# AlexIoannides/bodywork-mlops-demo

Measured on NVIDIA H100. Metric: train rows/sec (N x 128 least-squares fit), higher is better.
Workload: dtype bf16x2 (hi+lo) MMA operands, f32 accumulate, f64 fold+solve

## Files before the change

### bodywork-mlops-demo_b200/csrc/b2_internal.cuh

```cuda
#pragma once
#include <cuda.h>
#include <cuda_bf16.h>
#include <cuda_runtime.h>
#include <stdint.h>
#include <stdio.h>
#include <string.h>

#include <type_traits>

#include "../../include/b2gram.h"

namespace b2 {

constexpr int kMaxD = B2_MAX_D;
constexpr int kMaxS = kMaxD + 2;
constexpr int kKernelEventPairs = 64;
constexpr int kMaxRanks = 8;
constexpr size_t kXchgSlotDoubles = (size_t)kMaxS * kMaxS;
constexpr size_t kXchgDataDoubles = 2 * kMaxRanks * kXchgSlotDoubles;
constexpr size_t kXchgBytes = kXchgDataDoubles * sizeof(double) + 256;

constexpr int kTcRows = 64;
constexpr int kTcM = 128;
constexpr int kTcN = 144;
constexpr int kTcAccCols = 2 * kTcN;
constexpr int kTcAccElems = kTcM * kTcAccCols;
constexpr int kTcSums = 3;

constexpr int kNStats = 10;
constexpr int kGradOut = kMaxD + 1;
constexpr int kRfBeta = 0;
constexpr int kRfB0 = kMaxD;
constexpr int kRfMean = kMaxD + 1;
constexpr int kRfPrevBeta = 2 * kMaxD + 1;
constexpr int kRfPrevB0 = 3 * kMaxD + 1;
constexpr int kRfStep = 3 * kMaxD + 2;
constexpr int kRfGrad = 3 * kMaxD + 3;
constexpr int kRfDoubles = kRfGrad + kGradOut;
constexpr int kOutRefineStep = 2 * kMaxD + 3;
constexpr int kOutRefineGuard = 2 * kMaxD + 4;

inline int narrow_dp(int d) { return d <= 1 ? 1 : d <= 2 ? 2 : d <= 4 ? 4 : d <= 8 ? 8 : 16; }

void set_error(const char* fmt, ...);

#define B2_CUDA(call)                                                                      \
  do {                                                                                     \
    cudaError_t e_ = (call);                                                               \
    if (e_ != cudaSuccess) {                                                               \
// ... 132 lines not shown
```

### bodywork-mlops-demo_b200/csrc/gram_tc.cu

```cuda
#include <cuda_bf16.h>
#include <stdlib.h>

#include "b2_internal.cuh"
#include "b2_ptx.cuh"
#include "b2_shift.cuh"
#include "b2_xchg.cuh"

namespace b2 {
namespace {

constexpr int kConsumerWGs = 2;
constexpr int kXformWarps = 8;
constexpr int kThreads = 128 * (kConsumerWGs + 2);
constexpr int kFirstXformWarp = 4 * kConsumerWGs;
constexpr int kTmaWarp = kFirstXformWarp;
constexpr int kEWarp = kFirstXformWarp + 1;
static_assert(kFirstXformWarp + kXformWarps == kThreads / 32, "warp roles");
constexpr int kProducers = kXformWarps;
constexpr int kConsumerWarps = 4 * kConsumerWGs;
constexpr int kAccRegs = kTcN / 2;
constexpr int kKGroups = kTcRows / 8;
constexpr uint32_t kRawStageBytes = kTcRows * kMaxD * 4;
constexpr uint32_t kOpSBO = 128;
constexpr uint32_t kOpLBO = (16 + 2 + 16) * kOpSBO;
constexpr uint32_t kOpEOff = 16 * kOpSBO;
constexpr uint32_t kOpLoOff = 18 * kOpSBO;
constexpr uint32_t kOpStageBytes = kKGroups * kOpLBO;
constexpr int kMaxPack = 5;
constexpr uint32_t kYStageBytes = kTcRows * kMaxPack * 4;
constexpr uint32_t kMStageBytes = 384;
static_assert(kMStageBytes >= kTcRows * kMaxPack && kMStageBytes % 128 == 0 && kYStageBytes % 128 == 0, "stage alignment");

template <bool RAWB>
struct TcGeo {
  static constexpr int kRawStages = RAWB ? 4 : 3;
  static constexpr int kOpStages = RAWB ? 2 : 3;
  static constexpr int kAhead = RAWB ? kRawStages - 2 : kRawStages - 1;
  static constexpr uint32_t kOffRaw = 0;
  static constexpr uint32_t kOffOp = kOffRaw + kRawStages * kRawStageBytes;
  static constexpr uint32_t kOffY = kOffOp + kOpStages * kOpStageBytes;
  static constexpr uint32_t kOffMask = kOffY + kRawStages * kYStageBytes;
  static constexpr uint32_t kOffBar = kOffMask + kRawStages * kMStageBytes;
  static constexpr int kNumBars = 2 * kRawStages + 2 * kOpStages;
// ... 18 lines not shown
__device__ __forceinline__ void tma_load_1d(uint32_t dst, const CUtensorMap* tm, int c0, uint32_t bar) {
  asm volatile(
      "cp.async.bulk.tensor.1d.shared::cluster.global.mbarrier::complete_tx::bytes.L2::cache_hint"
      " [%0], [%1, {%3}], [%2], %4;" ::"r"(dst),
      "l"(reinterpret_cast<uint64_t>(tm)), "r"(bar), "r"(c0), "l"(kEvictFirst)
      : "memory");
}
__device__ __forceinline__ void tma_prefetch_desc(const CUtensorMap* tm) {
  asm volatile("prefetch.tensormap [%0];" ::"l"(reinterpret_cast<uint64_t>(tm)) : "memory");
}

__device__ __forceinline__ uint64_t make_smem_desc(uint32_t addr) {
  return (uint64_t)((addr & 0x3FFFFu) >> 4) | ((uint64_t)(kOpLBO >> 4) << 16) | ((uint64_t)(kOpSBO >> 4) << 32);
}
__device__ __forceinline__ void wgmma_fence() { asm volatile("wgmma.fence.sync.aligned;" ::: "memory"); }
__device__ __forceinline__ void wgmma_commit() { asm volatile("wgmma.commit_group.sync.aligned;" ::: "memory"); }
template <int N>
__device__ __forceinline__ void wgmma_wait() { asm volatile("wgmma.wait_group.sync.aligned %0;" ::"n"(N) : "memory"); }
template <int N>
__device__ __forceinline__ void fence_regs(float (&r)[N]) {
#pragma unroll
  for (int i = 0; i < N; ++i) asm volatile("" : "+f"(r[i])::"memory");
}
__device__ __forceinline__ void wgmma_m64n144k16(float (&d)[72], uint64_t adesc, uint64_t bdesc, uint32_t scale_d) {
  asm volatile(
      "{\n\t.reg .pred p;\n\t"
      "setp.ne.b32 p, %74, 0;\n\t"
      "wgmma.mma_async.sync.aligned.m64n144k16.f32.bf16.bf16 "
      "{%0, %1, %2, %3, %4, %5, %6, %7, %8, %9, %10, %11, "
      " %12, %13, %14, %15, %16, %17, %18, %19, %20, %21, %22, %23, "
      " %24, %25, %26, %27, %28, %29, %30, %31, %32, %33, %34, %35, "
      " %36, %37, %38, %39, %40, %41, %42, %43, %44, %45, %46, %47, "
      " %48, %49, %50, %51, %52, %53, %54, %55, %56, %57, %58, %59, "
      " %60, %61, %62, %63, %64, %65, %66, %67, %68, %69, %70, %71}, "
      "%72, %73, p, 1, 1, 0, 0;\n\t}"
      : "+f"(d[0]), "+f"(d[1]), "+f"(d[2]), "+f"(d[3]), "+f"(d[4]), "+f"(d[5]), "+f"(d[6]), "+f"(d[7]),
        "+f"(d[8]), "+f"(d[9]), "+f"(d[10]), "+f"(d[11]), "+f"(d[12]), "+f"(d[13]), "+f"(d[14]), "+f"(d[15]),
        "+f"(d[16]), "+f"(d[17]), "+f"(d[18]), "+f"(d[19]), "+f"(d[20]), "+f"(d[21]), "+f"(d[22]), "+f"(d[23]),
        "+f"(d[24]), "+f"(d[25]), "+f"(d[26]), "+f"(d[27]), "+f"(d[28]), "+f"(d[29]), "+f"(d[30]), "+f"(d[31]),
        "+f"(d[32]), "+f"(d[33]), "+f"(d[34]), "+f"(d[35]), "+f"(d[36]), "+f"(d[37]), "+f"(d[38]), "+f"(d[39]),
        "+f"(d[40]), "+f"(d[41]), "+f"(d[42]), "+f"(d[43]), "+f"(d[44]), "+f"(d[45]), "+f"(d[46]), "+f"(d[47]),
        "+f"(d[48]), "+f"(d[49]), "+f"(d[50]), "+f"(d[51]), "+f"(d[52]), "+f"(d[53]), "+f"(d[54]), "+f"(d[55]),
        "+f"(d[56]), "+f"(d[57]), "+f"(d[58]), "+f"(d[59]), "+f"(d[60]), "+f"(d[61]), "+f"(d[62]), "+f"(d[63]),
        "+f"(d[64]), "+f"(d[65]), "+f"(d[66]), "+f"(d[67]), "+f"(d[68]), "+f"(d[69]), "+f"(d[70]), "+f"(d[71])
      : "l"(adesc), "l"(bdesc), "r"(scale_d));
}
__device__ __forceinline__ void wgmma_m64n128k16_bmn(float* d, uint64_t adesc, uint64_t bdesc, uint32_t scale_d) {
  asm volatile(
      "{\n\t.reg .pred p;\n\t"
      "setp.ne.b32 p, %66, 0;\n\t"
      "wgmma.mma_async.sync.aligned.m64n128k16.f32.bf16.bf16 "
      "{%0, %1, %2, %3, %4, %5, %6, %7, %8, %9, %10, %11, %12, %13, %14, %15, "
      " %16, %17, %18, %19, %20, %21, %22, %23, %24, %25, %26, %27, %28, %29, %30, %31, "
      " %32, %33, %34, %35, %36, %37, %38, %39, %40, %41, %42, %43, %44, %45, %46, %47, "
      " %48, %49, %50, %51, %52, %53, %54, %55, %56, %57, %58, %59, %60, %61, %62, %63}, "
      "%64, %65, p, 1, 1, 0, 1;\n\t}"
      : "+f"(d[0]), "+f"(d[1]), "+f"(d[2]), "+f"(d[3]), "+f"(d[4]), "+f"(d[5]), "+f"(d[6]), "+f"(d[7]),
        "+f"(d[8]), "+f"(d[9]), "+f"(d[10]), "+f"(d[11]), "+f"(d[12]), "+f"(d[13]), "+f"(d[14]), "+f"(d[15]),
        "+f"(d[16]), "+f"(d[17]), "+f"(d[18]), "+f"(d[19]), "+f"(d[20]), "+f"(d[21]), "+f"(d[22]), "+f"(d[23]),
        "+f"(d[24]), "+f"(d[25]), "+f"(d[26]), "+f"(d[27]), "+f"(d[28]), "+f"(d[29]), "+f"(d[30]), "+f"(d[31]),
        "+f"(d[32]), "+f"(d[33]), "+f"(d[34]), "+f"(d[35]), "+f"(d[36]), "+f"(d[37]), "+f"(d[38]), "+f"(d[39]),
        "+f"(d[40]), "+f"(d[41]), "+f"(d[42]), "+f"(d[43]), "+f"(d[44]), "+f"(d[45]), "+f"(d[46]), "+f"(d[47]),
        "+f"(d[48]), "+f"(d[49]), "+f"(d[50]), "+f"(d[51]), "+f"(d[52]), "+f"(d[53]), "+f"(d[54]), "+f"(d[55]),
        "+f"(d[56]), "+f"(d[57]), "+f"(d[58]), "+f"(d[59]), "+f"(d[60]), "+f"(d[61]), "+f"(d[62]), "+f"(d[63])
      : "l"(adesc), "l"(bdesc), "r"(scale_d));
}
__device__ __forceinline__ void wgmma_m64n16k16(float* d, uint64_t adesc, uint64_t bdesc, uint32_t scale_d) {
  asm volatile(
      "{\n\t.reg .pred p;\n\t"
      "setp.ne.b32 p, %10, 0;\n\t"
      "wgmma.mma_async.sync.aligned.m64n16k16.f32.bf16.bf16 "
      "{%0, %1, %2, %3, %4, %5, %6, %7}, "
      "%8, %9, p, 1, 1, 0, 0;\n\t}"
      : "+f"(d[0]), "+f"(d[1]), "+f"(d[2]), "+f"(d[3]), "+f"(d[4]), "+f"(d[5]), "+f"(d[6]), "+f"(d[7])
      : "l"(adesc), "l"(bdesc), "r"(scale_d));
}
constexpr uint32_t kRawBoxBytes = kTcRows * 64 * 2;
__device__ __forceinline__ uint64_t make_raw_desc(uint32_t addr) {
  return (uint64_t)((addr & 0x3FFFFu) >> 4) | ((uint64_t)(kRawBoxBytes >> 4) << 16) | ((uint64_t)(1024u >> 4) << 32) |
         (1ull << 62);
}

__device__ __forceinline__ void st_shared_v4(uint32_t addr, const uint32_t (&v)[4]) {
  asm volatile("st.shared.v4.b32 [%0], {%1, %2, %3, %4};" ::"r"(addr), "r"(v[0]), "r"(v[1]), "r"(v[2]), "r"(v[3])
               : "memory");
}
__device__ __forceinline__ uint32_t lane_id() {
  uint32_t l;
  asm volatile("mov.u32 %0, %%laneid;" : "=r"(l));
  return l;
}
__device__ __forceinline__ void st_shared_f64(uint32_t addr, double v) {
  asm volatile("st.shared.f64 [%0], %1;" ::"r"(addr), "d"(v) : "memory");
}
__device__ __forceinline__ double ld_shared_f64(uint32_t addr) {
  double v;
  asm volatile("ld.shared.f64 %0, [%1];" : "=d"(v) : "r"(addr) : "memory");
  return v;
}
__device__ __forceinline__ void red_add_f64(double* p, double v) {
  asm volatile("red.global.add.f64 [%0], %1;" ::"l"(p), "d"(v) : "memory");
}
__device__ __forceinline__ void st_shared_u16(uint32_t addr, uint32_t v) {
  asm volatile("st.shared.u16 [%0], %1;" ::"r"(addr), "h"((unsigned short)v) : "memory");
}
__device__ __forceinline__ void split2(float v0, float v1, uint32_t& hi, uint32_t& lo) {
  const __nv_bfloat162 h = __floats2bfloat162_rn(v0, v1);
  hi = *reinterpret_cast<const uint32_t*>(&h);
  const float h0 = __uint_as_float(hi << 16), h1 = __uint_as_float(hi & 0xffff0000u);
  const __nv_bfloat162 l = __floats2bfloat162_rn(v0 - h0, v1 - h1);
  lo = *reinterpret_cast<const uint32_t*>(&l);
}

constexpr int kRedElems = kTcAccElems + kTcSums;

__device__ __forceinline__ void tc_reduce_range(const double* part, int n_ctas, double* red, int e0, int e1,
                                                double* quarter) {
  const int epb = blockDim.x >> 2;
  const int e = threadIdx.x % epb, q = threadIdx.x / epb;
  const int per = (n_ctas + 3) / 4;
  const int c0 = q * per, c1 = (c0 + per < n_ctas) ? c0 + per : n_ctas;
  for (int base = e0; base < e1; base += epb) {
    const int idx = base + e;
    if (idx < e1) {
      const bool sum = idx >= kTcAccElems;
      const double* src = sum ? part + (size_t)n_ctas * kTcAccElems + (idx - kTcAccElems) : part + idx;
      const size_t stride = sum ? kTcSums : kTcAccElems;
      double acc[8] = {0.0, 0.0, 0.0, 0.0, 0.0, 0.0, 0.0, 0.0};
      int c = c0;
      for (; c + 8 <= c1; c += 8) {
#pragma unroll
        for (int u = 0; u < 8; ++u) acc[u] += __ldcg(src + (size_t)(c + u) * stride);
      }
      for (; c < c1; ++c) acc[0] += __ldcg(src + (size_t)c * stride);
      quarter[q * epb + e] = ((acc[0] + acc[1]) + (acc[2] + acc[3])) + ((acc[4] + acc[5]) + (acc[6] + acc[7]));
    }
    __syncthreads();
    if (q == 0 && idx < e1) red[idx] = ((quarter[e] + quarter[epb + e]) + quarter[2 * epb + e]) + quarter[3 * epb + e];
    __syncthreads();
  }
}

__device__ __forceinline__ void grid_barrier(unsigned int* ctr) {
  __syncthreads();
  if (threadIdx.x == 0) {
    __threadfence();
    atomicAdd(ctr, 1u);
    const uint64_t t0 = globaltimer_ns();
    unsigned int seen;
    do {
      asm volatile("ld.acquire.gpu.global.u32 %0, [%1];" : "=r"(seen) : "l"(ctr) : "memory");
      if (seen < gridDim.x) {
        __nanosleep(40);
        if (globaltimer_ns() - t0 > 4000000000ull) __trap();
      }
    } while (seen < gridDim.x);
    __threadfence();
  }
  __syncthreads();
}

__device__ __forceinline__ double tc_fold_value(const double* red, const double* c, int d, int pack, int idx) {
  const int dp = d + 2;
  const int a = min(idx / dp, idx % dp), b = max(idx / dp, idx % dp);
  auto D1 = [&](int i, int j) { return __ldcg(red + (size_t)j * kTcM + i); };
  auto D2 = [&](int i, int j) { return __ldcg(red + (size_t)(kTcN + j) * kTcM + i); };
  auto s1 = [&](int i) {
    double t = 0.0;
    for (int blk = 0; blk < pack; ++blk) t += D1(blk * d + i, 128 + 3 * blk) + D2(blk * d + i, 128 + 3 * blk);
    return t;
  };
  auto sxy = [&](int i) {
    double t = 0.0;
    for (int blk = 0; blk < pack; ++blk) {
      const int r = blk * d + i, e = 128 + 3 * blk;
      t += D1(r, e + 1) + D1(r, e + 2) + D2(r, e + 1) + D2(r, e + 2);
    }
    return t;
  };
  auto G = [&](int i, int j) {
    double g = 0.0;
    for (int blk = 0; blk < pack; ++blk) {
      const int ia = blk * d + i, ib = blk * d + j;
      g += 0.5 * (D1(ia, ib) + D1(ib, ia)) + D2(ia, ib) + D2(ib, ia);
    }
    return g;
  };
  return unshift_entry(a, b, d, c, G, s1, sxy, __ldcg(red + kTcAccElems + 2), __ldcg(red + kTcAccElems + 0),
                       __ldcg(red + kTcAccElems + 1));
}

template <typename T, int DFIX, bool SPLIT, bool RAWB = false>
__global__ void __launch_bounds__(kThreads, 1)
gram_tc_kernel(const __grid_constant__ CUtensorMap tmX, const __grid_constant__ CUtensorMap tmY,
               const __grid_constant__ CUtensorMap tmM, int y_map_2d, int has_mask, int keep,
               int64_t n_rows, int d_arg, int pack, int d_orig, const float* __restrict__ shift,
               int chunk_tiles, double* __restrict__ part, uint32_t wait_ns, uint32_t dbg_arg) {
#ifdef B2_DEV_KNOBS
  const uint32_t dbg = dbg_arg;
#else
  constexpr uint32_t dbg = 0u;
  (void)dbg_arg;
#endif
  using G = TcGeo<RAWB>;
  constexpr int kRawStages = G::kRawStages, kOpStages = G::kOpStages;
  constexpr uint32_t kOffRaw = G::kOffRaw, kOffOp = G::kOffOp, kOffY = G::kOffY, kOffMask = G::kOffMask;
  const int d = DFIX ? DFIX : d_arg;
  extern __shared__ uint8_t smem_raw[];
  const uint32_t sbase = (smem_u32(smem_raw) + 1023u) & ~1023u;
  uint8_t* smem = smem_raw + (sbase - smem_u32(smem_raw));
  const int warp = threadIdx.x >> 5;
  const int lane = threadIdx.x & 31;

  const uint32_t bar_raw_full = sbase + G::kOffBar;
  const uint32_t bar_raw_empty = bar_raw_full + 8 * kRawStages;
// ... 11 lines not shown
      mbar_init(bar_raw_full + 8 * s, 1);
      mbar_init(bar_raw_empty + 8 * s, kProducers + (RAWB ? kConsumerWarps : 0));
    }
    for (int s = 0; s < kOpStages; ++s) {
      mbar_init(bar_op_full + 8 * s, kProducers);
      mbar_init(bar_op_empty + 8 * s, kConsumerWarps);
    }
    asm volatile("fence.mbarrier_init.release.cluster;" ::: "memory");
  }
  if (warp == kTmaWarp && lane == 0) {
    tma_prefetch_desc(&tmX);
    tma_prefetch_desc(&tmY);
    if (has_mask) tma_prefetch_desc(&tmM);
  }
  for (uint32_t o = threadIdx.x * 16; o < kOpStages * kOpStageBytes; o += kThreads * 16)
    *reinterpret_cast<uint4*>(smem + kOffOp + o) = make_uint4(0, 0, 0, 0);
  for (int j = threadIdx.x; j <= kMaxD; j += kThreads)
    shift_s[j] = j == kMaxD ? shift[kMaxD] : (j < pack * d_orig ? shift[j % d_orig] : 0.f);
  fence_proxy_async_smem();
  __syncthreads();

  if (warp < kConsumerWarps) {
    asm volatile("setmaxnreg.inc.sync.aligned.u32 %0;" ::"n"(G::kConsumerRegs));
    const int wg = warp >> 2;
    float acc1[kAccRegs], acc2[kAccRegs];
    double* my_part = part + (size_t)blockIdx.x * kTcAccElems + 64 * wg + 16 * (warp & 3) + (lane >> 2);
    auto store = [&](double* dst, bool add, auto val) {
#pragma unroll
      for (int r = 0; r < kAccRegs; ++r) {
        const int col = 8 * (r >> 2) + 2 * (lane & 3) + (r & 1), h = (r >> 1) & 1;
        const double v = val(r, col, h);
        double* p = dst + (size_t)col * kTcM + 8 * h;
        if (add) red_add_f64(p, v);
        else *p = v;
      }
    };
    auto drain = [&](const float (&acc)[kAccRegs], double* dst, bool add, double x_scale) {
      if constexpr (RAWB) {
        const double s1[2] = {(double)__shfl_sync(0xffffffffu, acc[64], lane & ~3),
                              (double)__shfl_sync(0xffffffffu, acc[66], lane & ~3)};
        store(dst, add, [&](int r, int col, int h) {
          return r < 64 ? x_scale * ((double)acc[r] - (double)shift_s[col] * s1[h]) : (double)acc[r];
        });
      } else {
        store(dst, add, [&](int r, int, int) { return (double)acc[r]; });
      }
    };
    auto release = [&](int tile) {
      mbar_arrive(bar_op_empty + 8 * (tile % kOpStages));
      if constexpr (RAWB) mbar_arrive(bar_raw_empty + 8 * (tile % kRawStages));
    };
    const uint32_t a_off = (uint32_t)wg * 8 * kOpSBO;
    int os = 0, held = -1, in_chunk = 0;
    uint32_t oph = 0;
    bool first_chunk = true;
    for (int it = 0; it < my_tiles; ++it) {
      mbar_wait(bar_op_full + 8 * os, oph, wait_ns);
      const uint32_t op_addr = sbase + kOffOp + os * kOpStageBytes;
      wgmma_fence();
#pragma unroll
      for (int k2 = 0; k2 < kTcRows / 16; ++k2) {
        const uint32_t k_addr = op_addr + k2 * 2 * kOpLBO;
        const uint64_t hi_desc = make_smem_desc(k_addr + a_off), lo_desc = make_smem_desc(k_addr + kOpLoOff + a_off);
        const uint32_t sc1 = (in_chunk > 0 || k2 > 0) ? 1u : 0u, sc2 = (it > 0 || k2 > 0) ? 1u : 0u;
        if constexpr (RAWB) {
          const uint64_t x_desc =
              make_raw_desc(sbase + kOffRaw + (uint32_t)(it % kRawStages) * kRawStageBytes + k2 * 16 * 128);
          const uint64_t e_desc = make_smem_desc(k_addr + kOpEOff);
          wgmma_m64n128k16_bmn(acc1, hi_desc, x_desc, sc1);
          wgmma_m64n16k16(acc1 + 64, hi_desc, e_desc, sc1);
          if constexpr (SPLIT) {
            wgmma_m64n128k16_bmn(acc2, lo_desc, x_desc, sc2);
            wgmma_m64n16k16(acc2 + 64, lo_desc, e_desc, sc2);
          }
        } else {
          const uint64_t b_desc = make_smem_desc(k_addr);
          if (!(dbg & 2u)) wgmma_m64n144k16(acc1, hi_desc, b_desc, sc1);
          if (SPLIT && !(dbg & 3u)) wgmma_m64n144k16(acc2, lo_desc, b_desc, sc2);
        }
      }
      wgmma_commit();
      const bool last = (in_chunk == chunk_tiles - 1) || (it == my_tiles - 1);
      if (last) {
        wgmma_wait<0>();
        fence_regs(acc1);
        if constexpr (SPLIT) fence_regs(acc2);
      } else {
        wgmma_wait<1>();
      }
      if (lane == 0) {
        if (held >= 0) release(held);
        if (last) release(it);
      }
      held = last ? -1 : it;
      if (last) {
        drain(acc1, my_part, !first_chunk, 1.0);
        first_chunk = false;
        in_chunk = 0;
      } else {
        ++in_chunk;
      }
      if (++os == kOpStages) { os = 0; oph ^= 1; }
    }
    wgmma_wait<0>();
    double* my_part2 = my_part + (size_t)kTcN * kTcM;
    if constexpr (SPLIT) {
      fence_regs(acc2);
      drain(acc2, my_part2, false, 0.5);
    } else {
      store(my_part2, false, [](int, int, int) { return 0.0; });
    }
  } else {
    asm volatile("setmaxnreg.dec.sync.aligned.u32 %0;" ::"n"(G::kProducerRegs));
    const uint32_t tx = (uint32_t)(kTcRows * d * sizeof(T)) + kTcRows * pack * 4 + (has_mask ? kTcRows * pack : 0);
    auto issue = [&](int j) {
      const int s = j % kRawStages;
      mbar_wait(bar_raw_empty + 8 * s, ((uint32_t)(j / kRawStages) & 1u) ^ 1u, wait_ns);
      const uint32_t full = bar_raw_full + 8 * s;
      mbar_expect_tx(full, tx);
      const int64_t row0 = (tile_begin + j) * kTcRows;
      tma_load_2d(sbase + kOffRaw + s * kRawStageBytes, &tmX, 0, (int)row0, full);
      if constexpr (RAWB) tma_load_2d(sbase + kOffRaw + s * kRawStageBytes + kRawBoxBytes, &tmX, 64, (int)row0, full);
      const int sub0 = (int)row0 * pack;
      if (y_map_2d) tma_load_2d(sbase + kOffY + s * kYStageBytes, &tmY, 0, sub0 >> 2, full);
      else tma_load_1d(sbase + kOffY + s * kYStageBytes, &tmY, sub0, full);
      if (has_mask == 2) tma_load_2d(sbase + kOffMask + s * kMStageBytes, &tmM, 0, sub0 >> 4, full);
      else if (has_mask) tma_load_1d(sbase + kOffMask + s * kMStageBytes, &tmM, sub0, full);
    };
    const bool issuer = warp == kTmaWarp && lane == 0;
    if (issuer)
      for (int j = 0; j < G::kAhead && j < my_tiles; ++j) issue(j);

    const int t = warp - kFirstXformWarp;
    const int nb = (d + 63) >> 6;
// ... 125 lines not shown
        syy += __shfl_xor_sync(0xffffffffu, syy, o);
        cnt += __shfl_xor_sync(0xffffffffu, cnt, o);
      }
      if (lane == 0) {
        double* ys = part + (size_t)gridDim.x * kTcAccElems + kTcSums * blockIdx.x;
        ys[0] = sy; ys[1] = syy; ys[2] = cnt;
      }
    }
  }
}

struct TcFinal {
  int assign;
  int n_ranks, rank;
  unsigned int epoch;
  PeerPtrs peers;
};

constexpr int kFinalizeThreads = 1024;
constexpr int kFinalizeCtas = (kRedElems + kFinalizeThreads / 4 - 1) / (kFinalizeThreads / 4);

__global__ void __launch_bounds__(kFinalizeThreads, 1)
tc_finalize_kernel(const double* part, int n_ctas, double* red, const float* __restrict__ shift, int d, int pack,
                   double* S, unsigned int* sync, const TcFinal fin) {
  __shared__ double quarter[kFinalizeThreads];
  __shared__ double c_s[kMaxD + 1];
  for (int j = threadIdx.x; j <= kMaxD; j += blockDim.x) c_s[j] = (double)shift[j];
  {
    constexpr int epb = kFinalizeThreads / 4;
    const int per = (((kRedElems + (int)gridDim.x - 1) / (int)gridDim.x) + epb - 1) / epb * epb;
    const int e0 = (int)blockIdx.x * per;
    const int e1 = e0 + per < kRedElems ? e0 + per : kRedElems;
    if (e0 < kRedElems) tc_reduce_range(part, n_ctas, red, e0, e1, quarter);
  }
  grid_barrier(sync + 0);
  {
    const int dp = d + 2;
    const int total = dp * dp;
    const size_t slot = xchg_slot_offset(fin.epoch, fin.rank);
    for (int idx = (int)(blockIdx.x * blockDim.x + threadIdx.x); idx < total; idx += (int)(gridDim.x * blockDim.x)) {
      const double val = tc_fold_value(red, c_s, d, pack, idx);
      const double sv = fin.assign ? val : S[idx] + val;
      S[idx] = sv;
      if (fin.n_ranks > 1) xchg_store_all(fin.peers, fin.n_ranks, slot, idx, sv);
    }
    if (fin.n_ranks > 1) __threadfence_system();
  }
  __syncthreads();
  __shared__ bool last_cta;
  if (threadIdx.x == 0) {
    __threadfence();
    last_cta = (atomicAdd(sync + 2, 1u) == gridDim.x - 1);
    if (last_cta) {
      sync[0] = 0u; sync[2] = 0u;
      __threadfence();
    }
  }
  __syncthreads();
  if (last_cta && fin.n_ranks > 1) xchg_publish(fin.peers, fin.n_ranks, fin.rank, fin.epoch);
}

typedef CUresult (*PFN_encodeTiled)(CUtensorMap*, CUtensorMapDataType, cuuint32_t, void*, const cuuint64_t*,
                                    const cuuint64_t*, const cuuint32_t*, const cuuint32_t*, CUtensorMapInterleave,
                                    CUtensorMapSwizzle, CUtensorMapL2promotion, CUtensorMapFloatOOBfill);
// ... 121 lines not shown

  const int64_t total_tiles = (n + kTcRows - 1) / kTcRows;
  const int sms = (ctx->sm_limit > 0 && ctx->sm_limit < ctx->sm_count) ? ctx->sm_limit : ctx->sm_count;
  const int grid = (int)(total_tiles < sms ? total_tiles : sms);
  int chunk_tiles = ctx->drain_rows / kTcRows / (rawb ? 4 : 1);
  if (chunk_tiles < 1) chunk_tiles = 1;

#ifdef B2_DEV_KNOBS
  static const uint32_t wait_ns = []() {
    const char* e = getenv("B2_WAIT_HINT_NS");
    return e ? (uint32_t)atoi(e) : 20000u;
  }();
#else
  constexpr uint32_t wait_ns = 20000u;
#endif
#ifdef B2_DEV_KNOBS
  static const uint32_t dbg = []() {
    const char* e = getenv("B2_TC_DEBUG");
    return e ? (uint32_t)atoi(e) : 0u;
  }();
#else
  constexpr uint32_t dbg = 0u;
#endif
  decltype(&gram_tc_kernel<float, 0, false>) kernel = nullptr;
  uint32_t smem = TcGeo<false>::kSmemBytes;
  with_rows(x_dtype, X, [&](auto* Xr) {
    using T = row_t<decltype(Xr)>;
    return with_int<0, 1>(ctx->precision == B2_PRECISION_SPLIT, [&](auto SP) {
      constexpr bool kSplit = decltype(SP)::value;
      kernel = d == 128 ? gram_tc_kernel<T, 128, kSplit> : gram_tc_kernel<T, 0, kSplit>;
      if constexpr (std::is_same_v<T, __nv_bfloat16>) {
        if (rawb) {
          kernel = gram_tc_kernel<T, 128, kSplit, true>;
          smem = TcGeo<true>::kSmemBytes;
        }
      }
      return B2_OK;
    });
  });
  B2_CUDA(cudaFuncSetAttribute(kernel, cudaFuncAttributeMaxDynamicSharedMemorySize, smem));
  const int pair = ctx->k_pairs % kKernelEventPairs;
  B2_CUDA(cudaEventRecord(ctx->ev_k[pair][0], ctx->stream));
  kernel<<<grid, kThreads, smem, ctx->stream>>>(tmX, tmY, tmM, tc.y_map_2d, mask != nullptr ? 1 + tc.m_map_2d : 0, keep,
                                                n, d, pack, d_in, ctx->shift, chunk_tiles, ctx->tc_part, wait_ns, dbg);
  B2_CUDA(cudaGetLastError());
  B2_CUDA(cudaEventRecord(ctx->ev_k[pair][1], ctx->stream));
  ctx->k_pairs += 1;

  TcFinal fin;
  memset(&fin, 0, sizeof(fin));
  fin.assign = assign ? 1 : 0;
  fin.n_ranks = 1;
  if (scatter_epoch != 0) {
    fin.n_ranks = ctx->n_ranks; fin.rank = ctx->rank; fin.epoch = scatter_epoch;
    for (int r = 0; r < kMaxRanks; ++r) fin.peers.p[r] = ctx->xchg_peer[r];
  }
  {
    cudaLaunchConfig_t cfg;
    memset(&cfg, 0, sizeof(cfg));
    cfg.gridDim = dim3(kFinalizeCtas < sms ? kFinalizeCtas : sms);
    cfg.blockDim = dim3(kFinalizeThreads); cfg.dynamicSmemBytes = 0; cfg.stream = ctx->stream;
    cudaLaunchAttribute attr[1];
    attr[0].id = cudaLaunchAttributeCooperative;
    attr[0].val.cooperative = 1;
    cfg.attrs = attr; cfg.numAttrs = 1;
    const double* part_arg = ctx->tc_part;
    const float* shift_arg = ctx->shift;
    B2_CUDA(cudaLaunchKernelEx(&cfg, tc_finalize_kernel, part_arg, grid, ctx->tc_red, shift_arg, d_in, pack, ctx->S,
                               ctx->tc_sync, fin));
  }
  ctx->launches += 2;
  return B2_OK;
}

}
```

Baseline: 4.143 billion.

## Exploit Gram symmetry: split consumer warpgroups into triangular MMA widths and pack partials

Each consumer warpgroup now issues WGMMA only over the columns at or above its row block (N=136/72 or 128/64 instead of 144 everywhere), and the extra-column width shrinks to 8 or 16 depending on pack. The per-CTA partial buffer is stored as a packed upper triangle plus extras, so drains write fewer doubles and the finalize reduction covers fewer elements. The aim is to cut redundant tensor-core work and global partial traffic on the symmetric X^T X. In exchange, the two warpgroups now do unequal amounts of work, the code adds more template instantiations, and the indexing becomes more complex, with risk of mistakes in the lower/upper fold logic.

```diff
diff --git a/bodywork-mlops-demo_b200/csrc/b2_internal.cuh b/bodywork-mlops-demo_b200/csrc/b2_internal.cuh
--- a/bodywork-mlops-demo_b200/csrc/b2_internal.cuh
+++ b/bodywork-mlops-demo_b200/csrc/b2_internal.cuh
@@ -22,9 +22,17 @@
 
 constexpr int kTcRows = 64;
 constexpr int kTcM = 128;
-constexpr int kTcN = 144;
-constexpr int kTcAccCols = 2 * kTcN;
-constexpr int kTcAccElems = kTcM * kTcAccCols;
+constexpr int kTcEMax = 16;
+inline int tc_e_width(int pack) { return pack >= 3 ? 16 : 8; }
+constexpr int kTcTri = kTcM * (kTcM + 1) / 2;
+__host__ __device__ constexpr int tc_part_index(int acc, int i, int j, int ew) {
+  return acc == 0 ? (j < kTcM ? j * (j + 1) / 2 + i : kTcTri + (j - kTcM) * kTcM + i)
+                  : kTcTri + ew * kTcM + j * kTcM + i;
+}
+__host__ __device__ constexpr int tc_part_elems(int ew, bool d2) {
+  return kTcTri + ew * kTcM + (d2 ? (kTcM + ew) * kTcM : 0);
+}
+constexpr int kTcAccElems = tc_part_elems(kTcEMax, true);
 constexpr int kTcSums = 3;
 
 constexpr int kNStats = 10;
diff --git a/bodywork-mlops-demo_b200/csrc/gram_tc.cu b/bodywork-mlops-demo_b200/csrc/gram_tc.cu
--- a/bodywork-mlops-demo_b200/csrc/gram_tc.cu
+++ b/bodywork-mlops-demo_b200/csrc/gram_tc.cu
@@ -18,7 +18,6 @@
 static_assert(kFirstXformWarp + kXformWarps == kThreads / 32, "warp roles");
 constexpr int kProducers = kXformWarps;
 constexpr int kConsumerWarps = 4 * kConsumerWGs;
-constexpr int kAccRegs = kTcN / 2;
 constexpr int kKGroups = kTcRows / 8;
 constexpr uint32_t kRawStageBytes = kTcRows * kMaxD * 4;
 constexpr uint32_t kOpSBO = 128;
@@ -83,59 +82,98 @@
 #pragma unroll
   for (int i = 0; i < N; ++i) asm volatile("" : "+f"(r[i])::"memory");
 }
-__device__ __forceinline__ void wgmma_m64n144k16(float (&d)[72], uint64_t adesc, uint64_t bdesc, uint32_t scale_d) {
+template <int N, int TB>
+__device__ __forceinline__ void wgmma(float* d, uint64_t adesc, uint64_t bdesc, uint32_t scale_d);
+#define B2_ACC4(o) "+f"(d[o]), "+f"(d[o + 1]), "+f"(d[o + 2]), "+f"(d[o + 3])
+#define B2_ACC8(o) B2_ACC4(o), B2_ACC4(o + 4)
+template <>
+__device__ __forceinline__ void wgmma<8, 0>(float* d, uint64_t adesc, uint64_t bdesc, uint32_t scale_d) {
   asm volatile(
-      "{\n\t.reg .pred p;\n\t"
-      "setp.ne.b32 p, %74, 0;\n\t"
+      "{\n\t.reg .pred p;\n\tsetp.ne.b32 p, %6, 0;\n\t"
+      "wgmma.mma_async.sync.aligned.m64n8k16.f32.bf16.bf16 "
+      "{%0, %1, %2, %3}, "
+      "%4, %5, p, 1, 1, 0, 0;\n\t}"
+      : B2_ACC4(0)
+      : "l"(adesc), "l"(bdesc), "r"(scale_d));
+}
+template <>
+__device__ __forceinline__ void wgmma<72, 0>(float* d, uint64_t adesc, uint64_t bdesc, uint32_t scale_d) {
+  asm volatile(
+      "{\n\t.reg .pred p;\n\tsetp.ne.b32 p, %38, 0;\n\t"
+      "wgmma.mma_async.sync.aligned.m64n72k16.f32.bf16.bf16 "
+      "{%0, %1, %2, %3, %4, %5, %6, %7, %8, %9, %10, %11, %12, %13, %14, %15, "
+      "%16, %17, %18, %19, %20, %21, %22, %23, %24, %25, %26, %27, %28, %29, %30, %31, "
+      "%32, %33, %34, %35}, "
+      "%36, %37, p, 1, 1, 0, 0;\n\t}"
+      : B2_ACC8(0), B2_ACC8(8), B2_ACC8(16), B2_ACC8(24), B2_ACC4(32)
+      : "l"(adesc), "l"(bdesc), "r"(scale_d));
+}
+template <>
+__device__ __forceinline__ void wgmma<80, 0>(float* d, uint64_t adesc, uint64_t bdesc, uint32_t scale_d) {
+  asm volatile(
+      "{\n\t.reg .pred p;\n\tsetp.ne.b32 p, %42, 0;\n\t"
+      "wgmma.mma_async.sync.aligned.m64n80k16.f32.bf16.bf16 "
+      "{%0, %1, %2, %3, %4, %5, %6, %7, %8, %9, %10, %11, %12, %13, %14, %15, "
+      "%16, %17, %18, %19, %20, %21, %22, %23, %24, %25, %26, %27, %28, %29, %30, %31, "
+      "%32, %33, %34, %35, %36, %37, %38, %39}, "
+      "%40, %41, p, 1, 1, 0, 0;\n\t}"
+      : B2_ACC8(0), B2_ACC8(8), B2_ACC8(16), B2_ACC8(24), B2_ACC8(32)
+      : "l"(adesc), "l"(bdesc), "r"(scale_d));
+}
+template <>
+__device__ __forceinline__ void wgmma<136, 0>(float* d, uint64_t adesc, uint64_t bdesc, uint32_t scale_d) {
+  asm volatile(
+      "{\n\t.reg .pred p;\n\tsetp.ne.b32 p, %70, 0;\n\t"
+      "wgmma.mma_async.sync.aligned.m64n136k16.f32.bf16.bf16 "
+      "{%0, %1, %2, %3, %4, %5, %6, %7, %8, %9, %10, %11, %12, %13, %14, %15, "
+      "%16, %17, %18, %19, %20, %21, %22, %23, %24, %25, %26, %27, %28, %29, %30, %31, "
+      "%32, %33, %34, %35, %36, %37, %38, %39, %40, %41, %42, %43, %44, %45, %46, %47, "
+      "%48, %49, %50, %51, %52, %53, %54, %55, %56, %57, %58, %59, %60, %61, %62, %63, "
+      "%64, %65, %66, %67}, "
+      "%68, %69, p, 1, 1, 0, 0;\n\t}"
+      : B2_ACC8(0), B2_ACC8(8), B2_ACC8(16), B2_ACC8(24), B2_ACC8(32), B2_ACC8(40), B2_ACC8(48), B2_ACC8(56), B2_ACC4(64)
+      : "l"(adesc), "l"(bdesc), "r"(scale_d));
+}
+template <>
+__device__ __forceinline__ void wgmma<144, 0>(float* d, uint64_t adesc, uint64_t bdesc, uint32_t scale_d) {
+  asm volatile(
+      "{\n\t.reg .pred p;\n\tsetp.ne.b32 p, %74, 0;\n\t"
       "wgmma.mma_async.sync.aligned.m64n144k16.f32.bf16.bf16 "
-      "{%0, %1, %2, %3, %4, %5, %6, %7, %8, %9, %10, %11, "
-      " %12, %13, %14, %15, %16, %17, %18, %19, %20, %21, %22, %23, "
-      " %24, %25, %26, %27, %28, %29, %30, %31, %32, %33, %34, %35, "
-      " %36, %37, %38, %39, %40, %41, %42, %43, %44, %45, %46, %47, "
-      " %48, %49, %50, %51, %52, %53, %54, %55, %56, %57, %58, %59, "
-      " %60, %61, %62, %63, %64, %65, %66, %67, %68, %69, %70, %71}, "
+      "{%0, %1, %2, %3, %4, %5, %6, %7, %8, %9, %10, %11, %12, %13, %14, %15, "
+      "%16, %17, %18, %19, %20, %21, %22, %23, %24, %25, %26, %27, %28, %29, %30, %31, "
+      "%32, %33, %34, %35, %36, %37, %38, %39, %40, %41, %42, %43, %44, %45, %46, %47, "
+      "%48, %49, %50, %51, %52, %53, %54, %55, %56, %57, %58, %59, %60, %61, %62, %63, "
+      "%64, %65, %66, %67, %68, %69, %70, %71}, "
       "%72, %73, p, 1, 1, 0, 0;\n\t}"
-      : "+f"(d[0]), "+f"(d[1]), "+f"(d[2]), "+f"(d[3]), "+f"(d[4]), "+f"(d[5]), "+f"(d[6]), "+f"(d[7]),
-        "+f"(d[8]), "+f"(d[9]), "+f"(d[10]), "+f"(d[11]), "+f"(d[12]), "+f"(d[13]), "+f"(d[14]), "+f"(d[15]),
-        "+f"(d[16]), "+f"(d[17]), "+f"(d[18]), "+f"(d[19]), "+f"(d[20]), "+f"(d[21]), "+f"(d[22]), "+f"(d[23]),
-        "+f"(d[24]), "+f"(d[25]), "+f"(d[26]), "+f"(d[27]), "+f"(d[28]), "+f"(d[29]), "+f"(d[30]), "+f"(d[31]),
-        "+f"(d[32]), "+f"(d[33]), "+f"(d[34]), "+f"(d[35]), "+f"(d[36]), "+f"(d[37]), "+f"(d[38]), "+f"(d[39]),
-        "+f"(d[40]), "+f"(d[41]), "+f"(d[42]), "+f"(d[43]), "+f"(d[44]), "+f"(d[45]), "+f"(d[46]), "+f"(d[47]),
-        "+f"(d[48]), "+f"(d[49]), "+f"(d[50]), "+f"(d[51]), "+f"(d[52]), "+f"(d[53]), "+f"(d[54]), "+f"(d[55]),
-        "+f"(d[56]), "+f"(d[57]), "+f"(d[58]), "+f"(d[59]), "+f"(d[60]), "+f"(d[61]), "+f"(d[62]), "+f"(d[63]),
-        "+f"(d[64]), "+f"(d[65]), "+f"(d[66]), "+f"(d[67]), "+f"(d[68]), "+f"(d[69]), "+f"(d[70]), "+f"(d[71])
+      : B2_ACC8(0), B2_ACC8(8), B2_ACC8(16), B2_ACC8(24), B2_ACC8(32), B2_ACC8(40), B2_ACC8(48), B2_ACC8(56), B2_ACC8(64)
       : "l"(adesc), "l"(bdesc), "r"(scale_d));
 }
-__device__ __forceinline__ void wgmma_m64n128k16_bmn(float* d, uint64_t adesc, uint64_t bdesc, uint32_t scale_d) {
+template <>
+__device__ __forceinline__ void wgmma<64, 1>(float* d, uint64_t adesc, uint64_t bdesc, uint32_t scale_d) {
   asm volatile(
-      "{\n\t.reg .pred p;\n\t"
-      "setp.ne.b32 p, %66, 0;\n\t"
+      "{\n\t.reg .pred p;\n\tsetp.ne.b32 p, %34, 0;\n\t"
+      "wgmma.mma_async.sync.aligned.m64n64k16.f32.bf16.bf16 "
+      "{%0, %1, %2, %3, %4, %5, %6, %7, %8, %9, %10, %11, %12, %13, %14, %15, "
+      "%16, %17, %18, %19, %20, %21, %22, %23, %24, %25, %26, %27, %28, %29, %30, %31}, "
+      "%32, %33, p, 1, 1, 0, 1;\n\t}"
+      : B2_ACC8(0), B2_ACC8(8), B2_ACC8(16), B2_ACC8(24)
+      : "l"(adesc), "l"(bdesc), "r"(scale_d));
+}
+template <>
+__device__ __forceinline__ void wgmma<128, 1>(float* d, uint64_t adesc, uint64_t bdesc, uint32_t scale_d) {
+  asm volatile(
+      "{\n\t.reg .pred p;\n\tsetp.ne.b32 p, %66, 0;\n\t"
       "wgmma.mma_async.sync.aligned.m64n128k16.f32.bf16.bf16 "
       "{%0, %1, %2, %3, %4, %5, %6, %7, %8, %9, %10, %11, %12, %13, %14, %15, "
-      " %16, %17, %18, %19, %20, %21, %22, %23, %24, %25, %26, %27, %28, %29, %30, %31, "
-      " %32, %33, %34, %35, %36, %37, %38, %39, %40, %41, %42, %43, %44, %45, %46, %47, "
-      " %48, %49, %50, %51, %52, %53, %54, %55, %56, %57, %58, %59, %60, %61, %62, %63}, "
+      "%16, %17, %18, %19, %20, %21, %22, %23, %24, %25, %26, %27, %28, %29, %30, %31, "
+      "%32, %33, %34, %35, %36, %37, %38, %39, %40, %41, %42, %43, %44, %45, %46, %47, "
+      "%48, %49, %50, %51, %52, %53, %54, %55, %56, %57, %58, %59, %60, %61, %62, %63}, "
       "%64, %65, p, 1, 1, 0, 1;\n\t}"
-      : "+f"(d[0]), "+f"(d[1]), "+f"(d[2]), "+f"(d[3]), "+f"(d[4]), "+f"(d[5]), "+f"(d[6]), "+f"(d[7]),
-        "+f"(d[8]), "+f"(d[9]), "+f"(d[10]), "+f"(d[11]), "+f"(d[12]), "+f"(d[13]), "+f"(d[14]), "+f"(d[15]),
-        "+f"(d[16]), "+f"(d[17]), "+f"(d[18]), "+f"(d[19]), "+f"(d[20]), "+f"(d[21]), "+f"(d[22]), "+f"(d[23]),
-        "+f"(d[24]), "+f"(d[25]), "+f"(d[26]), "+f"(d[27]), "+f"(d[28]), "+f"(d[29]), "+f"(d[30]), "+f"(d[31]),
-        "+f"(d[32]), "+f"(d[33]), "+f"(d[34]), "+f"(d[35]), "+f"(d[36]), "+f"(d[37]), "+f"(d[38]), "+f"(d[39]),
-        "+f"(d[40]), "+f"(d[41]), "+f"(d[42]), "+f"(d[43]), "+f"(d[44]), "+f"(d[45]), "+f"(d[46]), "+f"(d[47]),
-        "+f"(d[48]), "+f"(d[49]), "+f"(d[50]), "+f"(d[51]), "+f"(d[52]), "+f"(d[53]), "+f"(d[54]), "+f"(d[55]),
-        "+f"(d[56]), "+f"(d[57]), "+f"(d[58]), "+f"(d[59]), "+f"(d[60]), "+f"(d[61]), "+f"(d[62]), "+f"(d[63])
+      : B2_ACC8(0), B2_ACC8(8), B2_ACC8(16), B2_ACC8(24), B2_ACC8(32), B2_ACC8(40), B2_ACC8(48), B2_ACC8(56)
       : "l"(adesc), "l"(bdesc), "r"(scale_d));
 }
-__device__ __forceinline__ void wgmma_m64n16k16(float* d, uint64_t adesc, uint64_t bdesc, uint32_t scale_d) {
-  asm volatile(
-      "{\n\t.reg .pred p;\n\t"
-      "setp.ne.b32 p, %10, 0;\n\t"
-      "wgmma.mma_async.sync.aligned.m64n16k16.f32.bf16.bf16 "
-      "{%0, %1, %2, %3, %4, %5, %6, %7}, "
-      "%8, %9, p, 1, 1, 0, 0;\n\t}"
-      : "+f"(d[0]), "+f"(d[1]), "+f"(d[2]), "+f"(d[3]), "+f"(d[4]), "+f"(d[5]), "+f"(d[6]), "+f"(d[7])
-      : "l"(adesc), "l"(bdesc), "r"(scale_d));
-}
+#undef B2_ACC8
+#undef B2_ACC4
 constexpr uint32_t kRawBoxBytes = kTcRows * 64 * 2;
 __device__ __forceinline__ uint64_t make_raw_desc(uint32_t addr) {
   return (uint64_t)((addr & 0x3FFFFu) >> 4) | ((uint64_t)(kRawBoxBytes >> 4) << 16) | ((uint64_t)(1024u >> 4) << 32) |
@@ -159,8 +197,13 @@
   asm volatile("ld.shared.f64 %0, [%1];" : "=d"(v) : "r"(addr) : "memory");
   return v;
 }
-__device__ __forceinline__ void red_add_f64(double* p, double v) {
-  asm volatile("red.global.add.f64 [%0], %1;" ::"l"(p), "d"(v) : "memory");
+__device__ __forceinline__ void put_f64(double* p, double v, bool add, bool on) {
+  if (add)
+    asm volatile("{\n\t.reg .pred p;\n\tsetp.ne.b32 p, %2, 0;\n\t@p red.global.add.f64 [%0], %1;\n\t}"
+                 ::"l"(p), "d"(v), "r"((uint32_t)on) : "memory");
+  else
+    asm volatile("{\n\t.reg .pred p;\n\tsetp.ne.b32 p, %2, 0;\n\t@p st.global.f64 [%0], %1;\n\t}"
+                 ::"l"(p), "d"(v), "r"((uint32_t)on) : "memory");
 }
 __device__ __forceinline__ void st_shared_u16(uint32_t addr, uint32_t v) {
   asm volatile("st.shared.u16 [%0], %1;" ::"r"(addr), "h"((unsigned short)v) : "memory");
@@ -175,7 +218,7 @@
 
 constexpr int kRedElems = kTcAccElems + kTcSums;
 
-__device__ __forceinline__ void tc_reduce_range(const double* part, int n_ctas, double* red, int e0, int e1,
+__device__ __forceinline__ void tc_reduce_range(const double* part, int n_ctas, int n_acc, double* red, int e0, int e1,
                                                 double* quarter) {
   const int epb = blockDim.x >> 2;
   const int e = threadIdx.x % epb, q = threadIdx.x / epb;
@@ -183,9 +226,9 @@
   const int c0 = q * per, c1 = (c0 + per < n_ctas) ? c0 + per : n_ctas;
   for (int base = e0; base < e1; base += epb) {
     const int idx = base + e;
+    const bool sum = idx >= n_acc;
     if (idx < e1) {
-      const bool sum = idx >= kTcAccElems;
-      const double* src = sum ? part + (size_t)n_ctas * kTcAccElems + (idx - kTcAccElems) : part + idx;
+      const double* src = sum ? part + (size_t)n_ctas * kTcAccElems + (idx - n_acc) : part + idx;
       const size_t stride = sum ? kTcSums : kTcAccElems;
       double acc[8] = {0.0, 0.0, 0.0, 0.0, 0.0, 0.0, 0.0, 0.0};
       int c = c0;
@@ -197,7 +240,9 @@
       quarter[q * epb + e] = ((acc[0] + acc[1]) + (acc[2] + acc[3])) + ((acc[4] + acc[5]) + (acc[6] + acc[7]));
     }
     __syncthreads();
-    if (q == 0 && idx < e1) red[idx] = ((quarter[e] + quarter[epb + e]) + quarter[2 * epb + e]) + quarter[3 * epb + e];
+    if (q == 0 && idx < e1)
+      red[sum ? kTcAccElems + (idx - n_acc) : idx] =
+          ((quarter[e] + quarter[epb + e]) + quarter[2 * epb + e]) + quarter[3 * epb + e];
     __syncthreads();
   }
 }
@@ -221,21 +266,24 @@
   __syncthreads();
 }
 
-__device__ __forceinline__ double tc_fold_value(const double* red, const double* c, int d, int pack, int idx) {
+__device__ __forceinline__ double tc_fold_value(const double* red, const double* c, int d, int pack, int ew, bool d2,
+                                                int idx) {
   const int dp = d + 2;
   const int a = min(idx / dp, idx % dp), b = max(idx / dp, idx % dp);
-  auto D1 = [&](int i, int j) { return __ldcg(red + (size_t)j * kTcM + i); };
-  auto D2 = [&](int i, int j) { return __ldcg(red + (size_t)(kTcN + j) * kTcM + i); };
+  auto P = [&](int acc, int i, int j) { return __ldcg(red + tc_part_index(acc, i, j, ew)); };
   auto s1 = [&](int i) {
     double t = 0.0;
-    for (int blk = 0; blk < pack; ++blk) t += D1(blk * d + i, 128 + 3 * blk) + D2(blk * d + i, 128 + 3 * blk);
+    for (int blk = 0; blk < pack; ++blk) {
+      const int r = blk * d + i, e = kTcM + 3 * blk;
+      t += d2 ? P(0, r, e) + P(1, r, e) : P(0, r, e);
+    }
     return t;
   };
   auto sxy = [&](int i) {
     double t = 0.0;
     for (int blk = 0; blk < pack; ++blk) {
-      const int r = blk * d + i, e = 128 + 3 * blk;
-      t += D1(r, e + 1) + D1(r, e + 2) + D2(r, e + 1) + D2(r, e + 2);
+      const int r = blk * d + i, e = kTcM + 3 * blk;
+      t += d2 ? P(0, r, e + 1) + P(0, r, e + 2) + P(1, r, e + 1) + P(1, r, e + 2) : P(0, r, e + 1) + P(0, r, e + 2);
     }
     return t;
   };
@@ -243,7 +291,8 @@
     double g = 0.0;
     for (int blk = 0; blk < pack; ++blk) {
       const int ia = blk * d + i, ib = blk * d + j;
-      g += 0.5 * (D1(ia, ib) + D1(ib, ia)) + D2(ia, ib) + D2(ib, ia);
+      const double g1 = P(0, min(ia, ib), max(ia, ib));
+      g += d2 ? g1 + P(1, ia, ib) + P(1, ib, ia) : g1;
     }
     return g;
   };
@@ -251,7 +300,7 @@
                        __ldcg(red + kTcAccElems + 1));
 }
 
-template <typename T, int DFIX, bool SPLIT, bool RAWB = false>
+template <typename T, int DFIX, bool SPLIT, bool RAWB = false, int EW = 8>
 __global__ void __launch_bounds__(kThreads, 1)
 gram_tc_kernel(const __grid_constant__ CUtensorMap tmX, const __grid_constant__ CUtensorMap tmY,
                const __grid_constant__ CUtensorMap tmM, int y_map_2d, int has_mask, int keep,
@@ -309,94 +358,101 @@
 
   if (warp < kConsumerWarps) {
     asm volatile("setmaxnreg.inc.sync.aligned.u32 %0;" ::"n"(G::kConsumerRegs));
-    const int wg = warp >> 2;
-    float acc1[kAccRegs], acc2[kAccRegs];
-    double* my_part = part + (size_t)blockIdx.x * kTcAccElems + 64 * wg + 16 * (warp & 3) + (lane >> 2);
-    auto store = [&](double* dst, bool add, auto val) {
-#pragma unroll
-      for (int r = 0; r < kAccRegs; ++r) {
-        const int col = 8 * (r >> 2) + 2 * (lane & 3) + (r & 1), h = (r >> 1) & 1;
-        const double v = val(r, col, h);
-        double* p = dst + (size_t)col * kTcM + 8 * h;
-        if (add) red_add_f64(p, v);
-        else *p = v;
+    auto consume = [&](auto wg_c) {
+      constexpr int WG = decltype(wg_c)::value;
+      constexpr int kF1 = kTcM - 64 * WG;
+      constexpr int kF2 = RAWB ? kF1 : kTcM;
+      constexpr int kC1 = 64 * WG;
+      constexpr int kR1 = (kF1 + EW) / 2, kR2 = (kF2 + EW) / 2;
+      float acc1[kR1], acc2[kR2];
+      double* my_part = part + (size_t)blockIdx.x * kTcAccElems;
+      auto store = [&](auto n_regs, int dst_acc, int col0, bool add, auto val) {
+        const int ln = (int)lane_id(), row0 = 64 * WG + 16 * (warp & 3) + (ln >> 2);
+#pragma unroll
+        for (int r = 0; r < decltype(n_regs)::value; ++r) {
+          const int col = col0 + 8 * (r >> 2) + 2 * (ln & 3) + (r & 1), h = (r >> 1) & 1, i = row0 + 8 * h;
+          const bool lower = dst_acc == 0 && col < kTcM && i > col;
+          put_f64(my_part + tc_part_index(dst_acc, i, col, EW), val(r, col, h), add, !lower);
+        }
+      };
+      auto drain = [&](const auto& acc, int dst_acc, int col0, bool add) {
+        constexpr int kR = sizeof(acc) / sizeof(float);
+        if constexpr (RAWB) {
+          constexpr int kF = 2 * kR - EW;
+          const double s1[2] = {(double)__shfl_sync(0xffffffffu, acc[kF / 2], lane & ~3),
+                                (double)__shfl_sync(0xffffffffu, acc[kF / 2 + 2], lane & ~3)};
+          store(std::integral_constant<int, kR>{}, dst_acc, col0, add, [&](int r, int col, int h) {
+            return col < kTcM ? (double)acc[r] - (double)shift_s[col] * s1[h] : (double)acc[r];
+          });
+        } else {
+          store(std::integral_constant<int, kR>{}, dst_acc, col0, add, [&](int r, int, int) { return (double)acc[r]; });
+        }
+      };
+      auto release = [&](int tile) {
+        mbar_arrive(bar_op_empty + 8 * (tile % kOpStages));
+        if constexpr (RAWB) mbar_arrive(bar_raw_empty + 8 * (tile % kRawStages));
+      };
+      constexpr uint32_t a_off = (uint32_t)WG * 8 * kOpSBO;
+      int os = 0, held = -1, in_chunk = 0;
+      uint32_t oph = 0;
+      bool first_chunk = true;
+      for (int it = 0; it < my_tiles; ++it) {
+        mbar_wait(bar_op_full + 8 * os, oph, wait_ns);
+        const uint32_t op_addr = sbase + kOffOp + os * kOpStageBytes;
+        wgmma_fence();
+#pragma unroll
+        for (int k2 = 0; k2 < kTcRows / 16; ++k2) {
+          const uint32_t k_addr = op_addr + k2 * 2 * kOpLBO;
+          const uint64_t hi_desc = make_smem_desc(k_addr + a_off), lo_desc = make_smem_desc(k_addr + kOpLoOff + a_off);
+          const uint32_t sc1 = (in_chunk > 0 || k2 > 0) ? 1u : 0u, sc2 = (it > 0 || k2 > 0) ? 1u : 0u;
+          if constexpr (RAWB) {
+            const uint64_t x_desc = make_raw_desc(sbase + kOffRaw + (uint32_t)(it % kRawStages) * kRawStageBytes +
+                                                  (uint32_t)WG * kRawBoxBytes + k2 * 16 * 128);
+            const uint64_t e_desc = make_smem_desc(k_addr + kOpEOff);
+            if (!(dbg & 2u)) {
+              wgmma<kF1, 1>(acc1, hi_desc, x_desc, sc1);
+              wgmma<EW, 0>(acc1 + kF1 / 2, hi_desc, e_desc, sc1);
+            }
+            if (SPLIT && !(dbg & 3u)) {
+              wgmma<kF2, 1>(acc2, lo_desc, x_desc, sc2);
+              wgmma<EW, 0>(acc2 + kF2 / 2, lo_desc, e_desc, sc2);
+            }
+          } else {
+            if (!(dbg & 2u)) wgmma<kF1 + EW, 0>(acc1, hi_desc, make_smem_desc(k_addr + a_off), sc1);
+            if (SPLIT && !(dbg & 3u)) wgmma<kF2 + EW, 0>(acc2, lo_desc, make_smem_desc(k_addr), sc2);
+          }
+        }
+        wgmma_commit();
+        const bool last = (in_chunk == chunk_tiles - 1) || (it == my_tiles - 1);
+        if (last) {
+          wgmma_wait<0>();
+          fence_regs(acc1);
+          if constexpr (SPLIT) fence_regs(acc2);
+        } else {
+          wgmma_wait<1>();
+        }
+        if (lane == 0) {
+          if (held >= 0) release(held);
+          if (last) release(it);
+        }
+        held = last ? -1 : it;
+        if (last) {
+          drain(acc1, 0, kC1, !first_chunk);
+          first_chunk = false;
+          in_chunk = 0;
+        } else {
+          ++in_chunk;
+        }
+        if (++os == kOpStages) { os = 0; oph ^= 1; }
+      }
+      wgmma_wait<0>();
+      if constexpr (SPLIT) {
+        fence_regs(acc2);
+        drain(acc2, RAWB ? 0 : 1, RAWB ? kC1 : 0, RAWB);
       }
     };
-    auto drain = [&](const float (&acc)[kAccRegs], double* dst, bool add, double x_scale) {
-      if constexpr (RAWB) {
-        const double s1[2] = {(double)__shfl_sync(0xffffffffu, acc[64], lane & ~3),
-                              (double)__shfl_sync(0xffffffffu, acc[66], lane & ~3)};
-        store(dst, add, [&](int r, int col, int h) {
-          return r < 64 ? x_scale * ((double)acc[r] - (double)shift_s[col] * s1[h]) : (double)acc[r];
-        });
-      } else {
-        store(dst, add, [&](int r, int, int) { return (double)acc[r]; });
-      }
-    };
-    auto release = [&](int tile) {
-      mbar_arrive(bar_op_empty + 8 * (tile % kOpStages));
-      if constexpr (RAWB) mbar_arrive(bar_raw_empty + 8 * (tile % kRawStages));
-    };
-    const uint32_t a_off = (uint32_t)wg * 8 * kOpSBO;
-    int os = 0, held = -1, in_chunk = 0;
-    uint32_t oph = 0;
-    bool first_chunk = true;
-    for (int it = 0; it < my_tiles; ++it) {
-      mbar_wait(bar_op_full + 8 * os, oph, wait_ns);
-      const uint32_t op_addr = sbase + kOffOp + os * kOpStageBytes;
-      wgmma_fence();
-#pragma unroll
-      for (int k2 = 0; k2 < kTcRows / 16; ++k2) {
-        const uint32_t k_addr = op_addr + k2 * 2 * kOpLBO;
-        const uint64_t hi_desc = make_smem_desc(k_addr + a_off), lo_desc = make_smem_desc(k_addr + kOpLoOff + a_off);
-        const uint32_t sc1 = (in_chunk > 0 || k2 > 0) ? 1u : 0u, sc2 = (it > 0 || k2 > 0) ? 1u : 0u;
-        if constexpr (RAWB) {
-          const uint64_t x_desc =
-              make_raw_desc(sbase + kOffRaw + (uint32_t)(it % kRawStages) * kRawStageBytes + k2 * 16 * 128);
-          const uint64_t e_desc = make_smem_desc(k_addr + kOpEOff);
-          wgmma_m64n128k16_bmn(acc1, hi_desc, x_desc, sc1);
-          wgmma_m64n16k16(acc1 + 64, hi_desc, e_desc, sc1);
-          if constexpr (SPLIT) {
-            wgmma_m64n128k16_bmn(acc2, lo_desc, x_desc, sc2);
-            wgmma_m64n16k16(acc2 + 64, lo_desc, e_desc, sc2);
-          }
-        } else {
-          const uint64_t b_desc = make_smem_desc(k_addr);
-          if (!(dbg & 2u)) wgmma_m64n144k16(acc1, hi_desc, b_desc, sc1);
-          if (SPLIT && !(dbg & 3u)) wgmma_m64n144k16(acc2, lo_desc, b_desc, sc2);
-        }
-      }
-      wgmma_commit();
-      const bool last = (in_chunk == chunk_tiles - 1) || (it == my_tiles - 1);
-      if (last) {
-        wgmma_wait<0>();
-        fence_regs(acc1);
-        if constexpr (SPLIT) fence_regs(acc2);
-      } else {
-        wgmma_wait<1>();
-      }
-      if (lane == 0) {
-        if (held >= 0) release(held);
-        if (last) release(it);
-      }
-      held = last ? -1 : it;
-      if (last) {
-        drain(acc1, my_part, !first_chunk, 1.0);
-        first_chunk = false;
-        in_chunk = 0;
-      } else {
-        ++in_chunk;
-      }
-      if (++os == kOpStages) { os = 0; oph ^= 1; }
-    }
-    wgmma_wait<0>();
-    double* my_part2 = my_part + (size_t)kTcN * kTcM;
-    if constexpr (SPLIT) {
-      fence_regs(acc2);
-      drain(acc2, my_part2, false, 0.5);
-    } else {
-      store(my_part2, false, [](int, int, int) { return 0.0; });
-    }
+    if (__shfl_sync(0xffffffffu, warp, 0) >= 4) consume(std::integral_constant<int, 1>{});
+    else consume(std::integral_constant<int, 0>{});
   } else {
     asm volatile("setmaxnreg.dec.sync.aligned.u32 %0;" ::"n"(G::kProducerRegs));
     const uint32_t tx = (uint32_t)(kTcRows * d * sizeof(T)) + kTcRows * pack * 4 + (has_mask ? kTcRows * pack : 0);
@@ -568,16 +624,18 @@
 
 __global__ void __launch_bounds__(kFinalizeThreads, 1)
 tc_finalize_kernel(const double* part, int n_ctas, double* red, const float* __restrict__ shift, int d, int pack,
-                   double* S, unsigned int* sync, const TcFinal fin) {
+                   int ew, int d2, double* S, unsigned int* sync, const TcFinal fin) {
   __shared__ double quarter[kFinalizeThreads];
   __shared__ double c_s[kMaxD + 1];
   for (int j = threadIdx.x; j <= kMaxD; j += blockDim.x) c_s[j] = (double)shift[j];
   {
     constexpr int epb = kFinalizeThreads / 4;
-    const int per = (((kRedElems + (int)gridDim.x - 1) / (int)gridDim.x) + epb - 1) / epb * epb;
+    const int n_acc = tc_part_elems(ew, d2 != 0);
+    const int n_red = n_acc + kTcSums;
+    const int per = (((n_red + (int)gridDim.x - 1) / (int)gridDim.x) + epb - 1) / epb * epb;
     const int e0 = (int)blockIdx.x * per;
-    const int e1 = e0 + per < kRedElems ? e0 + per : kRedElems;
-    if (e0 < kRedElems) tc_reduce_range(part, n_ctas, red, e0, e1, quarter);
+    const int e1 = e0 + per < n_red ? e0 + per : n_red;
+    if (e0 < n_red) tc_reduce_range(part, n_ctas, n_acc, red, e0, e1, quarter);
   }
   grid_barrier(sync + 0);
   {
@@ -585,7 +643,7 @@
     const int total = dp * dp;
     const size_t slot = xchg_slot_offset(fin.epoch, fin.rank);
     for (int idx = (int)(blockIdx.x * blockDim.x + threadIdx.x); idx < total; idx += (int)(gridDim.x * blockDim.x)) {
-      const double val = tc_fold_value(red, c_s, d, pack, idx);
+      const double val = tc_fold_value(red, c_s, d, pack, ew, d2 != 0, idx);
       const double sv = fin.assign ? val : S[idx] + val;
       S[idx] = sv;
       if (fin.n_ranks > 1) xchg_store_all(fin.peers, fin.n_ranks, slot, idx, sv);
@@ -753,13 +811,18 @@
 #else
   constexpr uint32_t dbg = 0u;
 #endif
+  const bool split = ctx->precision == B2_PRECISION_SPLIT;
+  const int ew = tc_e_width(pack);
+  const bool d2 = split && !rawb;
   decltype(&gram_tc_kernel<float, 0, false>) kernel = nullptr;
   uint32_t smem = TcGeo<false>::kSmemBytes;
   with_rows(x_dtype, X, [&](auto* Xr) {
     using T = row_t<decltype(Xr)>;
-    return with_int<0, 1>(ctx->precision == B2_PRECISION_SPLIT, [&](auto SP) {
+    return with_int<0, 1>(split, [&](auto SP) {
       constexpr bool kSplit = decltype(SP)::value;
-      kernel = d == 128 ? gram_tc_kernel<T, 128, kSplit> : gram_tc_kernel<T, 0, kSplit>;
+      if (d != 128) kernel = gram_tc_kernel<T, 0, kSplit>;
+      else if (ew == 16) kernel = gram_tc_kernel<T, 128, kSplit, false, 16>;
+      else kernel = gram_tc_kernel<T, 128, kSplit>;
       if constexpr (std::is_same_v<T, __nv_bfloat16>) {
         if (rawb) {
           kernel = gram_tc_kernel<T, 128, kSplit, true>;
@@ -797,8 +860,8 @@
     cfg.attrs = attr; cfg.numAttrs = 1;
     const double* part_arg = ctx->tc_part;
     const float* shift_arg = ctx->shift;
-    B2_CUDA(cudaLaunchKernelEx(&cfg, tc_finalize_kernel, part_arg, grid, ctx->tc_red, shift_arg, d_in, pack, ctx->S,
-                               ctx->tc_sync, fin));
+    B2_CUDA(cudaLaunchKernelEx(&cfg, tc_finalize_kernel, part_arg, grid, ctx->tc_red, shift_arg, d_in, pack, ew,
+                               d2 ? 1 : 0, ctx->S, ctx->tc_sync, fin));
   }
   ctx->launches += 2;
   return B2_OK;
```

Result: faster. 4.511 billion (median of 6 runs) (+8.9%).
